# Amandaynzhou/MMT-PSM

Hardware: AMD Instinct MI355X
Metric: imgs/sec (student+teacher step, 1000x1000, AUG_K=2) (higher is better)
Workload: dtype f32

## Files before the change

### include/mmtpsm.h

```cpp
#ifndef MMTPSM_H
#define MMTPSM_H
#include <stdint.h>
#ifdef __cplusplus
extern "C" {
#endif

#define MMT_EINVAL (-22)

int mmt_version(void);

typedef struct {
  const float* feat[4];
  float* grad_feat[4];
  int H[4];
  int W[4];
  float scale[4];
  int num_levels;
  int N;
  int C;
} mmt_pyramid;

int mmt_roi_align_forward(const mmt_pyramid* pyr , const float* rois, const int32_t* levels,
                          int K, int PH, int PW, int sampling_ratio, float* out, void* stream);
int mmt_roi_align_forward_bf16(const mmt_pyramid* pyr , const float* rois, const int32_t* levels,
// ... 147 lines not shown
                          const void* dy_planes, long dy_plane_stride, const float* s_x, const float* s_dy, const float* rowscale,
                          float* dw, float* dbias, float* workspace, void* stream);
typedef struct {
  void* fn;
  long a[16];
} mmt_call;
int mmt_replay(const mmt_call* calls , int n, int* failed_index );
int mmt_split_planes_f16_rb(const float* x, void* planes, long plane_stride, int rows, int W, int C, const float* amax,
                            float* scale_out, void* stream);
int mmt_conv_writes_rb(const mmt_conv_args* a );
typedef struct mmt_wgrad_job {
  mmt_conv_args a;
  const float* dy; const float* rowscale; float* dw; float* dbias;
  const void* x_planes; long x_plane_stride; const void* dy_planes; long dy_plane_stride; const float* s_x; const float* s_dy;
} mmt_wgrad_job;
int mmt_conv_wgrad_group_workspace(const mmt_wgrad_job* jobs , int n, long* floats_out );
int mmt_conv_wgrad_group(const mmt_wgrad_job* jobs , int n, float* workspace, long workspace_floats, void* stream);
int mmt_sum_stats_rb(const float* a, const float* b, const float* c, const float* d, float* y, int rows, int W, int C, float* slot,
                     void* planes, long plane_stride, const float* scale, float* amax_next, void* stream);
int mmt_rb_scales_update(float* state, int n, void* stream);
int mmt_conv_forward_pg(const mmt_conv_args* a , const float* s_x , const float* s_w , int tile_rows,
                        int ksplit, void* stream);
int mmt_conv_pg_plan(const mmt_conv_args* a , int* tile_rows, int* ksplit);
int mmt_conv_pg_wanted(const mmt_conv_args* a );
typedef struct { long src_off, dst_off; int Cout, K, unit0, pad; } mmt_pack_desc;
long mmt_packed_weight_elems(int Cout, int K);
int mmt_pack_weight(const float* w, void* planes, long plane_stride, int Cout, int K, void* stream);
int mmt_pack_weight_flipped(const float* w, const float* scale, void* planes, long plane_stride, int Cout, int KH, int KW,
                            int Cin, void* stream);
int mmt_split_planes(const float* x, void* planes, long plane_stride, long n, void* stream);
typedef struct { const float* w; const float* scale; void* dst; long plane_stride; int Cout, KH, KW, Cin, unit0, pad; } mmt_flip_desc;
int mmt_pack_weights_flipped(const mmt_flip_desc* descs , const int* unit_desc , int n_units, void* stream);
int mmt_pack_weights(const float* base, void* planes, long plane_stride, const mmt_pack_desc* descs ,
                     const int* unit_desc , int n_units, void* stream);
int mmt_pack_weights_f16(const float* base, void* planes, long plane_stride, const mmt_pack_desc* descs ,
                         const int* unit_desc , int n_units, int n_descs, float* stat , void* stream);
int mmt_pack_weights_flipped_f16(const mmt_flip_desc* descs , const int* unit_desc , int n_units, int n_descs,
                                 float* stat , void* stream);

int mmt_conv_wgrad_splits(const mmt_conv_args* a );
int mmt_conv_wgrad(const mmt_conv_args* a , const float* dy,
                   const float* rowscale , float* dw, float* dbias ,
                   float* workspace , void* stream);

int mmt_colsum(const float* dy, int M, int C, float* out, void* stream);

// ... 41 lines not shown
```

### mmt-psm_amd/csrc/conv_igemm.hip

```cpp
#include <stdlib.h>
#include <map>
#include <mutex>
#include <type_traits>
#include "conv_shared.h"

namespace {

template <int BM, int BN, int WM, int WN>
__device__ __forceinline__ void conv_epilogue_stage(f32x16 (&acc)[BM / (32 * WM)][BN / (32 * WN)], float* lds,
                                                    const int lane, const int wm, const int wn) {
  constexpr int TM = BM / (32 * WM), TN = BN / (32 * WN);
  float* ct = lds;
  const int col_l = lane & 31, rq = lane >> 5;
#pragma unroll
  for (int a = 0; a < TM; a++)
#pragma unroll
    for (int b = 0; b < TN; b++)
#pragma unroll
      for (int r = 0; r < 16; r++) {
        const int row = (wm * TM + a) * 32 + (r & 3) + 8 * (r >> 2) + 4 * rq;
        ct[row * BN + (wn * TN + b) * 32 + col_l] = acc[a][b][r];
      }
}

// ... 1793 lines not shown
    }
    return MMT_EINVAL;
  }
  if (ksplit > 1) return launch_glds<128, 128, 4, 1, NS, 3>(p, s, ksplit);
  switch (variant) {
    case 1: return launch_glds<128, 128, 4, 1, NS, 3>(p, s);
    case 3: return launch_glds<128, 64, 4, 1, NS, 3>(p, s);
    default: return launch_glds<64, 64, 2, 2, NS, 3>(p, s);
  }
}

template <int NS>
int launch_split_variant(int variant, const ConvP& p, hipStream_t s) {
  switch (variant) {
    case 1: return launch_split<128, 128, 2, 2, NS>(p, s);
    case 3: return launch_split<128, 64, 2, 2, NS>(p, s);
    default: return launch_split<64, 64, 2, 2, NS>(p, s);
  }
}

}

namespace mmtconv {
static int g_precision = -1;
int precision() {
  if (g_precision < 0) {
    g_precision = getenv("MMT_CONV_PRECISION") ? atoi(getenv("MMT_CONV_PRECISION")) : 3;
    if (g_precision < 0 || g_precision > 3) g_precision = 3;
  }
  return g_precision;
}
}

extern "C" int mmt_set_conv_precision(int mode) {
  if (mode < 0 || mode > 3) return MMT_EINVAL;
  mmtconv::g_precision = mode;
  return 0;
}

extern "C" int mmt_get_conv_precision(void) { return precision(); }

extern "C" int mmt_conv3x3_strip_f16x2(const mmt_conv_args* a, const float* s_x, const float* s_w, void* stream) {
  ConvP p;
  int e = fill(p, a);
  if (e) return e;
  if (!p.y || !p.xpl || !p.wpl || !s_x || !s_w || p.io || p.ypl) return MMT_EINVAL;
// ... 45 lines not shown
extern "C" int mmt_conv_forward_f16x2(const mmt_conv_args* a, const float* x_amax, const float* s_w, void* stream) {
  ConvP p;
  int e = fill(p, a);
  if (e) return e;
  if (!p.y || !p.wpl || !x_amax || !s_w || p.io || p.ypl || p.xpl_rb || (p.Cin & 15) || ((size_t)p.wpl & 15) || (p.wpl_stride & 7)) return MMT_EINVAL;
  if (p.M == 0 || p.Cout == 0) return 0;
  const int variant = pick_variant(p);
  if (variant == 0) return MMT_EINVAL;
  p.f16_sx = x_amax; p.f16_sw = s_w; p.f16_ax = 1;
  hipStream_t s = (hipStream_t)stream;
  if (p.yrb && !rb_epilogue_ok(p)) return MMT_EINVAL;
  if (c64_shape(p)) return launch_c64(p, s);
  if (rows_shape(p, true)) {
    if (p.mask) {
      if (p.Cin == 64) return launch_rows<4, 2, true, true>(p, s);
      if (p.Cin == 128) return launch_rows<8, 2, true, true>(p, s);
      return launch_rows<16, 2, true, true>(p, s);
    }
    if (p.Cin == 64) return launch_rows<4, 2, true>(p, s);
    if (p.Cin == 128) return launch_rows<8, 2, true>(p, s);
    return launch_rows<16, 2, true>(p, s);
  }
  const int ksplit = pick_ksplit(p);
  constexpr int S = 3;
  auto go = [&](auto kern, int BM, int BN, int ks) -> int {
    const int tiles = mmt_cdiv(p.M, BM) * mmt_cdiv(p.Cout, BN) * ks;
    SplitWs w{nullptr, nullptr};
    if (ks > 1) {
      w = split_workspace(s);
      if (!w.ws || tiles > 1024) return MMT_EINVAL;
    }
    const size_t ring = (size_t)S * (BM * 64 + 2 * BN * 32), epi = (size_t)BM * BN * sizeof(float);
    const size_t lds = ring > epi ? ring : epi;
    if (lds > 65536) {
      const hipError_t er = hipFuncSetAttribute((const void*)kern, hipFuncAttributeMaxDynamicSharedMemorySize, (int)lds);
      if (er != hipSuccess) return (int)er;
    }
    hipLaunchKernelGGL(kern, dim3(tiles), dim3(256), lds, s, p, p.wpl, p.wpl_stride, ks, w.ws);
    if (ks > 1)
      launch_finish<128, 128>(p, tiles / ks, ks, w.ws, s);
    return 0;
  };
#define MMT_GLDS_GO(SS)                                                                                      \
  do {                                                                                                       \
    if (ksplit > 1) e = go(conv_fwd_glds_kernel<128, 128, 4, 1, 2, SS, true>, 128, 128, ksplit);            \
    else if (variant == 1) e = go(conv_fwd_glds_kernel<128, 128, 4, 1, 2, SS, true>, 128, 128, 1);          \
// ... 1 lines not shown
    else e = go(conv_fwd_glds_kernel<64, 64, 2, 2, 2, SS, true>, 64, 64, 1);                                \
  } while (0)
  MMT_GLDS_GO(3);
#undef MMT_GLDS_GO
  if (e) return e;
  MMT_LAUNCH_CHECK();
  return 0;
}

static int pick_variant(const ConvP& p) {
  if (p.Cout <= 32) return 0;
  constexpr int lowk = 256;
  constexpr int lowv = 3;
  if (p.K <= lowk) return (p.Cout >= 64 && (long)mmt_cdiv(p.M, 128) * mmt_cdiv(p.Cout, 64) >= 768) ? lowv : 2;
  const long t128 = (long)mmt_cdiv(p.M, 128) * mmt_cdiv(p.Cout, 128);
  constexpr int t128min = 256;
  if (t128 >= t128min && p.Cout > 64) return 1;
  constexpr int mid = 1;
  const long t12864 = (long)mmt_cdiv(p.M, 128) * mmt_cdiv(p.Cout, 64);
  if (mid && t12864 >= 256 && p.Cout >= 64) return 3;
  return 2;
}

extern "C" int mmt_conv_variant(const mmt_conv_args* a) {
  ConvP p;
  int e = fill(p, a);
  if (e) return e;
  const int v = pick_variant(p);
  if (v != 0 && (precision() == 3 || (precision() == 1 && (p.io & IO_X))) && strip_tw(p)) return 4;
  if (v != 0 && precision() > 0 && (p.Cin & 15) == 0 && p.wpl && pick_ksplit(p) > 1) return 1;
  return v;
}

extern "C" int mmt_conv_wants_planes(const mmt_conv_args* a) {
  ConvP p;
  int e = fill(p, a);
  if (e) return 0;
  if (precision() != 3 || pick_variant(p) == 0) return 0;
  return strip_tw(p, false) ? 1 : 0;
}

extern "C" int mmt_conv_ksplit(const mmt_conv_args* a) {
  ConvP p;
  int e = fill(p, a);
  if (e) return e;
  if (pick_variant(p) != 0 && (precision() == 3 || (precision() == 1 && (p.io & IO_X))) && strip_tw(p)) return 1;
  if (pick_variant(p) != 0 && precision() > 0 && (p.Cin & 15) == 0 && p.wpl) return pick_ksplit(p);
  return 1;
}

// ... 30 lines not shown
```

### mmt-psm_amd/csrc/conv_pgemm.hip

```cpp
#include <map>
#include <mutex>
#include "conv_shared.h"

namespace {

constexpr unsigned PG_OOB = 0x80000000u;

template <int I, int U, class F>
__device__ __forceinline__ void pg_unroll(F&& f) {
  if constexpr (I < U) {
    f(std::integral_constant<int, I>{});
    pg_unroll<I + 1, U>(f);
  }
}

template <int WM, int KG, int S, int DBG = 0, bool AF = false>
__global__ __launch_bounds__(768) void conv_pg_kernel(const ConvP p, const int ksplit, float* __restrict__ ws,
                                                      unsigned* __restrict__ tickets) {
  constexpr int BM = 64 * WM, BN = 128, GW = 2 * WM, NT = 512, GT = 64 * GW, NTALL = 768;
  static_assert(GW * KG == 8, "eight matrix waves");
  constexpr int PA = BM * 32, PB = BN * 32;
  constexpr int A_BYTES = 2 * PA, GSTAGE = A_BYTES + 2 * PB, STAGE = KG * GSTAGE;
  constexpr int PPG = 4 / KG, NBP = 8 / PPG, NI = 4 + NBP;
  constexpr int U = (S % 2) ? 2 * S : S;
  constexpr int OWN = 4 / KG;
  static_assert(S >= 3 && (S - 2) * NI < 64, "ring depth / vmcnt range");
  extern __shared__ __attribute__((aligned(16))) float lds[];
  char* const ring = (char*)lds;
  const int tid = threadIdx.x, lane = tid & 63;
  const int wave = __builtin_amdgcn_readfirstlane(tid >> 6);
  const bool copier = wave >= 8;
  const int cw = wave - 8;
  const int grp = copier ? cw / PPG : wave / GW;
  const int gwave = wave % GW;
  const int wm = gwave >> 1, wn = gwave & 1;
  const int gtid = tid - grp * GT;

  const int tiles_n = (p.Cout + BN - 1) / BN;
  int bid = blockIdx.x;
  {
    const int nwg = gridDim.x, q = nwg >> 3, r = nwg & 7, xcd = bid & 7, idx = bid >> 3;
    bid = (xcd < r ? xcd * (q + 1) : r * (q + 1) + (xcd - r) * q) + idx;
  }
  const int ks = bid % ksplit;
  bid /= ksplit;
  const int tile_lin = bid;
  const int tile_m = bid / tiles_n, tile_n = bid % tiles_n;
  const int m0 = tile_m * BM, n0 = tile_n * BN;
  const int HoWo = p.Ho * p.Wo;
  const F16Guard guard = f16_guard_load(p.guard_x);
  const float s_lag = p.xpl_lag ? *p.f16_sx : 0.f;
  auto guard_bad = [&]() { return p.xpl_lag ? f16_guard_bad_lag(guard, s_lag) : f16_guard_bad(guard); };

  const int nkt_all = p.K >> 4, spt = p.Cin >> 4;
  const int R = ksplit * KG, rng = ks * KG + grp;
  const int kt0 = (int)((long)rng * nkt_all / R), nkt = (int)((long)(rng + 1) * nkt_all / R) - kt0;
  const int nkt_max = (nkt_all + R - 1) / R;
  char* const gring = ring + grp * GSTAGE;

  f32x16 acc[2][2];
#pragma unroll
  for (int a = 0; a < 2; a++)
#pragma unroll
    for (int b = 0; b < 2; b++)
#pragma unroll
      for (int r = 0; r < 16; r++) acc[a][b][r] = 0.f;

  if (copier) {
    const int sub = cw % PPG;
    const int ar = (DBG & 64) ? lane >> 3 : (DBG & 32) ? lane >> 2 : lane >> 1;
    const int alh = (DBG & 64) ? (lane & 7) : (DBG & 32) ? (lane & 3) : (lane & 1) ^ ((ar >> 3) & 1);
    int aih0[2], aiw0[2];
    unsigned apix[2];
    bool aok[2];
#pragma unroll
    for (int t = 0; t < 2; t++) {
      const int m = m0 + (2 * sub + t) * 32 + ar;
      aok[t] = m < p.M;
      const int mm = aok[t] ? m : 0;
      const int img = mm / HoWo, rem = mm - img * HoWo;
      const int ho = rem / p.Wo, wo = rem - ho * p.Wo;
      aih0[t] = ho * p.stride - p.pad;
      aiw0[t] = wo * p.stride - p.pad;
      apix[t] = (unsigned)img * (unsigned)(p.H * p.W);
    }
    const long n_x = (long)p.N * p.H * p.W * p.Cin;
    const __amdgpu_buffer_rsrc_t rs_a0 = AF ? __builtin_amdgcn_make_buffer_rsrc((void*)p.x, 0, (int)(n_x * 4), 0x00020000)
                                            : __builtin_amdgcn_make_buffer_rsrc((void*)p.xpl, 0, (int)(n_x * 2), 0x00020000);
    const __amdgpu_buffer_rsrc_t rs_a1 = AF ? rs_a0
                                            : __builtin_amdgcn_make_buffer_rsrc((void*)(p.xpl + p.xpl_stride), 0, (int)(n_x * 2), 0x00020000);
    const __amdgpu_buffer_rsrc_t rs_b = __builtin_amdgcn_make_buffer_rsrc((void*)p.wpl, 0, 0x7ffffff0, 0x00020000);
    const int nb32 = (p.Cout + 31) >> 5;
    const int b_step = nb32 * 1024;
    unsigned vo_b[NBP];
    int dst_b[NBP];
#pragma unroll
    for (int i = 0; i < NBP; i++) {
      const int t = NBP * sub + i, q = t >> 2, cb = t & 3;
      int nb = n0 / 32 + cb;
      if (nb >= nb32) nb = nb32 - 1;
      vo_b[i] = (unsigned)((q * p.wpl_stride + (long)nb * 512 + lane * 8) * 2);
      dst_b[i] = A_BYTES + q * PB + cb * 1024;
    }
    int f_kh, f_kw, f_ci, f_n = 0;
    {
      const int tap0 = kt0 / spt;
      f_ci = kt0 - tap0 * spt;
      f_kh = tap0 / p.KW;
      f_kw = tap0 - f_kh * p.KW;
    }
    const int a_step = AF ? 64 : (p.xpl_rb ? p.W * 32 : 32);
    int soff_a = f_ci * a_step, soff_b = kt0 * b_step;
    unsigned vo_a[2] = {PG_OOB, PG_OOB};
    auto enter_tap = [&]() {
#pragma unroll
      for (int t = 0; t < 2; t++) {
        const int ih = aih0[t] + f_kh, iw = aiw0[t] + f_kw;
        const bool ok = aok[t] && (unsigned)ih < (unsigned)p.H && (unsigned)iw < (unsigned)p.W;
        vo_a[t] = !ok ? PG_OOB
                  : AF ? ((apix[t] + (unsigned)(ih * p.W + iw)) * (unsigned)p.Cin + (unsigned)(alh * 8)) * 4u
                  : p.xpl_rb ? (((apix[t] + (unsigned)(ih * p.W)) * (unsigned)spt + (unsigned)iw) * 16u + (unsigned)(alh * 8)) * 2u
                             : ((apix[t] + (unsigned)(ih * p.W + iw)) * (unsigned)p.Cin + (unsigned)(alh * 8)) * 2u;
      }
    };
    enter_tap();
    auto advance = [&]() {
      f_n++;
      if constexpr (DBG & 1) { soff_b += (DBG & 2) ? 0 : b_step; return; }
      soff_a += a_step;
      soff_b += (DBG & 2) ? 0 : b_step;
      if (++f_ci == spt) {
        f_ci = 0;
        soff_a = 0;
        if (++f_kw == p.KW) { f_kw = 0; ++f_kh; }
        enter_tap();
      }
    };
    auto copy_step = [&](int stage) {
      const bool real = (DBG & 4) ? false : f_n < nkt;
      char* const st = gring + stage * STAGE;
#pragma unroll
      for (int t = 0; t < 2; t++) {
        const int va = (int)(real ? vo_a[t] : PG_OOB);
        __builtin_amdgcn_raw_ptr_buffer_load_lds(rs_a0, (lds_ptr_t)(st + (2 * sub + t) * 1024), 16, va, soff_a, 0, 0);
        __builtin_amdgcn_raw_ptr_buffer_load_lds(rs_a1, (lds_ptr_t)(st + PA + (2 * sub + t) * 1024), 16, va, soff_a, 0, 0);
      }
#pragma unroll
      for (int i = 0; i < NBP; i++)
        __builtin_amdgcn_raw_ptr_buffer_load_lds(rs_b, (lds_ptr_t)(st + dst_b[i]), 16, (int)(real ? vo_b[i] : PG_OOB), soff_b, 0, 0);
      advance();
    };
    auto wait_copies = [&]() {
      asm volatile("s_waitcnt vmcnt(%0)" ::"n"((S - 2) * NI) : "memory");
    };
    if constexpr (AF || (DBG & 16)) {
      typedef unsigned u32x4 __attribute__((ext_vector_type(4)));
      u32x4 rg[S][NI];
      const float s_a = AF ? f16_scale_of(*p.f16_sx) : 1.f;
      auto load_step = [&](auto setc) {
        constexpr int set = decltype(setc)::value;
        const bool real = f_n < nkt;
#pragma unroll
        for (int t = 0; t < 2; t++) {
          const int va = (int)(real ? vo_a[t] : PG_OOB);
          rg[set][2 * t] = __builtin_amdgcn_raw_buffer_load_b128(rs_a0, va, soff_a, 0);
          rg[set][2 * t + 1] = __builtin_amdgcn_raw_buffer_load_b128(rs_a1, AF ? va + 16 : va, soff_a, 0);
        }
#pragma unroll
// ... 82 lines not shown
        default: fa[1][1] = *(const f16x8*)(a + PA + 1024); break;
      }
    };
    auto step = [&](int kt, int st_next, const f16x8 (&fa)[2][2], const f16x8 (&fb)[2][2], f16x8 (&fan)[2][2], f16x8 (&fbn)[2][2]) {
      asm volatile("s_waitcnt lgkmcnt(0)" ::: "memory");
      __builtin_amdgcn_s_barrier();
      if (kt < nkt) {
        int j = 0;
#pragma unroll
        for (int pr = 0; pr < 3; pr++) {
          const int qa = pr == 1 ? 1 : 0, qb = pr == 0 ? 1 : 0;
#pragma unroll
          for (int a = 0; a < 2; a++)
#pragma unroll
            for (int b = 0; b < 2; b++) {
              acc[a][b] = __builtin_amdgcn_mfma_f32_32x32x16_f16(fa[qa][a], fb[qb][b], acc[a][b], 0, 0, 0);
              if (j < 8) { if constexpr (!(DBG & 8)) fread(j, st_next, fan, fbn); }
              j++;
              __builtin_amdgcn_sched_barrier(0);
            }
        }
      }
    };
    if (!guard_bad()) {
      __builtin_amdgcn_s_barrier();
      f16x8 faP[2][2], fbP[2][2], faQ[2][2], fbQ[2][2];
#pragma unroll
      for (int i = 0; i < 8; i++) fread(i, 0, faP, fbP);
      if constexpr (DBG & 8) {
#pragma unroll
        for (int i = 0; i < 8; i++) fread(i, 1, faQ, fbQ);
      }
      for (int kt = 0; kt < nkt_max; kt += U) {
        pg_unroll<0, U>([&](auto ic) {
          constexpr int i = decltype(ic)::value;
          if (i == 0 || kt + i < nkt_max) {
            if constexpr (i % 2 == 0) step(kt + i, (i + 1) % S, faP, fbP, faQ, fbQ);
            else step(kt + i, (i + 1) % S, faQ, fbQ, faP, fbP);
          }
        });
      }
    }
    asm volatile("s_waitcnt lgkmcnt(0)" ::: "memory");
  }
  if (guard_bad()) {
    if (ks == 0) conv_slow_tile(m0, BM, 0, BM, n0, BN, nullptr, false, tid, NTALL, blockIdx.x);
    return;
// ... 74 lines not shown
            u32x4 t[4];
#pragma unroll
            for (int r4 = 0; r4 < 4; r4++) t[r4] = __builtin_amdgcn_raw_buffer_load_b128(rws, (int)(slab_off + (unsigned)((o * 4 + r4) * NT * 16)), 0, 16);
#pragma unroll
            for (int r4 = 0; r4 < 4; r4++) {
              const f32x4 v = __builtin_bit_cast(f32x4, t[r4]);
#pragma unroll
              for (int c = 0; c < 4; c++) {
                if (j == 0) acc[i >> 1][i & 1][4 * r4 + c] = v[c]; else acc[i >> 1][i & 1][4 * r4 + c] += v[c];
              }
            }
            o++;
          }
        }
      }
    }
  }

  {
    const int mrow0 = m0 + wm * 64 + 4 * (lane >> 5);
    conv_epilogue_direct<2, 2>(p, acc, (unsigned)mrow0 * ((unsigned)p.Cout * 4u), p.M - mrow0, n0 + wn * 64 + (lane & 31),
                         copier ? 0 : (KG == 1 ? 15 : (KG == 2 ? (grp ? 10 : 5) : (1 << grp))), (float*)ring + 64, wave, lane, tid, blockIdx.x);
  }
}

__global__ __launch_bounds__(256) void split_planes_f16_rb_kernel(const float* __restrict__ x, unsigned short* __restrict__ pl,
                                                                  const long plane_stride, const int W, const int C, const int segs,
                                                                  const float* __restrict__ amax, float* __restrict__ s_out) {
  constexpr int CBS = 1024 + 32;
  __shared__ __attribute__((aligned(16))) char tile[2 * 16 * CBS];
  const float s = f16_scale_of(*amax);
  if (blockIdx.x == 0 && blockIdx.y == 0 && threadIdx.x == 0 && s_out) *s_out = s;
  const int row = blockIdx.x / segs, w0 = (blockIdx.x % segs) * 32, c0 = blockIdx.y * 256;
  const int cc = min(256, C - c0), c4n = cc >> 2, ncb = cc >> 4, npx = min(32, W - w0);
  const float* const src = x + ((long)row * W + w0) * C + c0;
  const int total = npx * c4n;
  f32x4 v[8];
#pragma unroll
  for (int u = 0; u < 8; u++) {
    const int i = threadIdx.x + 256 * u;
    const int px = i / c4n, c4 = i - px * c4n;
    v[u] = i < total ? ldg4(src + (long)px * C + c4 * 4) : f32x4{0.f, 0.f, 0.f, 0.f};
  }
#pragma unroll
  for (int u = 0; u < 8; u++) {
    const int i = threadIdx.x + 256 * u;
// ... 122 lines not shown

bool pg_shape(const ConvP& p) {
  return p.xpl && p.wpl && !p.io && !p.ypl && !p.mul && p.out_stride == 1 && p.res_mode <= 1 && (p.Cin & 15) == 0 && p.Cout > 32 &&
         (long)p.N * p.H * p.W * p.Cin < (1L << 29) && (long)p.M * p.Cout * 4 < (1L << 31) && ((size_t)p.xpl & 15) == 0 &&
         (p.xpl_stride & 7) == 0 && ((size_t)p.wpl & 15) == 0 && (p.wpl_stride & 7) == 0;
}

void pg_plan(const ConvP& p, int& rows, int& ksplit) {
  const long tn = mmt_cdiv(p.Cout, 128);
  const long t256 = (long)mmt_cdiv(p.M, 256) * tn, t128 = (long)mmt_cdiv(p.M, 128) * tn, t64 = (long)mmt_cdiv(p.M, 64) * tn;
  const int nkt = p.K >> 4;
  rows = t256 >= 448 ? 256 : (t128 >= 224 ? 128 : 64);
  ksplit = 1;
  if (rows == 64 && t64 <= 128) {
    int ks = (int)(256 / t64);
    if (ks > nkt / 64) ks = nkt / 64;
    if (ks > 8) ks = 8;
    if (ks >= 2) ksplit = ks;
  }
  const char* e = getenv("MMT_SPLITK");
  if (e && atoi(e) == 0) ksplit = 1;
}

template <int WM, int KG, int S, int DBG = 0, bool AF = false>
int launch_pg(const ConvP& p, hipStream_t s, int ksplit) {
  constexpr int BM = 64 * WM;
  const int tiles = mmt_cdiv(p.M, BM) * mmt_cdiv(p.Cout, 128);
  SplitWs w{nullptr, nullptr};
  if (ksplit > 1) {
    w = split_workspace(s);
    if (!w.ws || !w.tickets || tiles > SPLITK_TICKETS || (size_t)tiles * ksplit * BM * 128 * 4 > SPLITK_WS_BYTES) return MMT_EINVAL;
  }
  constexpr size_t ring = (size_t)S * KG * (BM * 64 + 2 * 128 * 32), xch = KG > 1 ? (size_t)4 * (KG - 1) * 4 * (128 * WM) * 16 : 0;
  constexpr size_t lds = ring > xch ? ring : xch;
  static_assert(lds <= 160 * 1024, "LDS");
  auto kern = conv_pg_kernel<WM, KG, S, DBG, AF>;
  static bool done = false;
  if (!done) {
    const hipError_t e = hipFuncSetAttribute((const void*)kern, hipFuncAttributeMaxDynamicSharedMemorySize, (int)lds);
    if (e != hipSuccess) return (int)e;
    done = true;
  }
  hipLaunchKernelGGL(kern, dim3(tiles * ksplit), dim3(768), lds, s, p, ksplit, w.ws, w.tickets);
  MMT_LAUNCH_CHECK();
  return 0;
}

}

extern "C" int mmt_conv_pg_plan(const mmt_conv_args* a, int* tile_rows, int* ksplit) {
  ConvP p;
  int e = fill(p, a);
  if (e) return e;
  int rows = 0, ks = 0;
  if (precision() == 3 && p.wpl && p.M > 0 && p.Cout > 0) {
    const unsigned short* keep = p.xpl;
    if (!p.xpl) p.xpl = (const unsigned short*)16;
    if (pg_shape(p)) pg_plan(p, rows, ks);
    p.xpl = keep;
  }
  if (tile_rows) *tile_rows = rows;
  if (ksplit) *ksplit = ks;
  return 0;
}

extern "C" int mmt_conv_pg_wanted(const mmt_conv_args* a) {
  ConvP p;
  if (fill(p, a)) return 0;
  if (precision() != 3 || !p.wpl || p.M <= 0 || p.Cout < 96 || p.KH * p.KW < 4) return 0;
  const char* e = getenv("MMT_PG");
// ... 82 lines not shown
      case 8: return launch_pg<1, 4, 3, 8>(p, s, ks);
      case 12: return launch_pg<1, 4, 3, 12>(p, s, ks);
      default: break;
    }
    if (rows == 256) switch (dbg) {
      case 1: return launch_pg<4, 1, 4, 1>(p, s, ks);
      case 2: return launch_pg<4, 1, 4, 2>(p, s, ks);
      case 4: return launch_pg<4, 1, 4, 4>(p, s, ks);
      case 8: return launch_pg<4, 1, 4, 8>(p, s, ks);
      case 12: return launch_pg<4, 1, 4, 12>(p, s, ks);
      default: break;
    }
  }
#endif
  if (af) {
#ifdef MMT_PG_ABLATE
    if (rows == 256) return launch_pg<4, 1, 4, 0, true>(p, s, ks);
    if (rows == 128) return launch_pg<2, 2, 4, 0, true>(p, s, ks);
    return launch_pg<1, 4, 3, 0, true>(p, s, ks);
#else
    return MMT_EINVAL;
#endif
  }
  if (rows == 256) return launch_pg<4, 1, 4>(p, s, ks);
  if (rows == 128) return launch_pg<2, 2, 4>(p, s, ks);
  return launch_pg<1, 4, 3>(p, s, ks);
}
```

### mmt-psm_amd/csrc/conv_shared.h

```cpp
#pragma once
#include <stdlib.h>
#include <type_traits>
#include "common.h"

namespace mmtconv {

struct ConvP {
  const float* x; const float* w; const float* scale; const float* shift; const float* res;
  const float* mask; const float* mul; float* y;
  int N, H, W, Cin, Cout, KH, KW, stride, pad, Ho, Wo;
  int relu, res_mode, out_stride, out_H, out_W;
  float mask_scale;
  int M, K, cin32, cin4;
  const unsigned short* wpl; long wpl_stride;
  const unsigned short* xpl; long xpl_stride;
  unsigned short* ypl; long ypl_stride;
  unsigned* amax_out;
  int amax_stats;
  int f16_ax;
  const float* f16_sx; const float* f16_sw;
  int io;
  const float* guard_x; const float* guard_dy;
  const float* w_src; const float* w_src_scale;
  const float* x2; const float* dy2; const float* f16_sx2; const float* f16_sw2; const float* guard_x2; const float* guard_dy2;
// ... 1 lines not shown
  int staged_epilogue;
  int xpl_rb;
  unsigned short* yrb; long yrb_stride; const float* yrb_s; unsigned* amax_next; int xpl_lag;
  int yrb_M;
};
constexpr float F16_CREST_HI = 131072.f;
constexpr int IO_X = 1, IO_Y = 2, IO_RES = 4, IO_MASK = 8, IO_DY = 16;

int fill(ConvP& p, const mmt_conv_args* a);
int precision();
struct SplitWs { float* ws; unsigned* tickets; };
constexpr size_t SPLITK_WS_BYTES = (size_t)1024 * 128 * 128 * 4;
constexpr int SPLITK_TICKETS = 4096;
SplitWs split_workspace(hipStream_t s);
struct WgReduceItem { const float* ws; const float* rowscale; float* dw; int splits, Cout, NP, pad; };
int launch_wgrad_reduce_group(const WgReduceItem* items, int n, hipStream_t s);
struct WgPlJob { const mmt_conv_args* a; const float* dy; const void* xpl; long xpl_stride; const void* dpl; long dpl_stride;
                 const float* s_x; const float* s_dy; const float* rowscale; float* dw; float* dbias; float* ws; int ksplit; };
int wgpl_eligible_splits(const mmt_conv_args* a);
long wgpl_super_steps(const mmt_conv_args* a);
int launch_wgpl_group(const WgPlJob* jobs, int n, hipStream_t s);
bool c64_shape(const ConvP& p);
int launch_c64(const ConvP& p, hipStream_t s);
}

namespace {
using namespace mmtconv;

struct F16Guard { float amax, s0, s1, s2, s3, c0, c1, c2, c3; };
__device__ __forceinline__ F16Guard f16_guard_load(const float* __restrict__ slot) {
  F16Guard g = {0.f, 0.f, 0.f, 0.f, 0.f, 0.f, 0.f, 0.f, 0.f};
  if (slot) { g.amax = slot[0]; g.s0 = slot[1]; g.s1 = slot[2]; g.s2 = slot[3]; g.s3 = slot[4];
              g.c0 = slot[17]; g.c1 = slot[18]; g.c2 = slot[19]; g.c3 = slot[20]; }
  return g;
}
__device__ __forceinline__ bool f16_guard_bad(const F16Guard& g) {
  const float tot = (g.s0 + g.s1) + (g.s2 + g.s3), cnt = (g.c0 + g.c1) + (g.c2 + g.c3);
  if (!(tot > 0.f)) return false;
  if (!(g.amax == g.amax) || g.amax > 3.0e38f) return true;
  return g.amax * cnt > tot * F16_CREST_HI;
}

__device__ __forceinline__ bool f16_guard_bad_lag(const F16Guard& g, const float s) {
  const float tot = (g.s0 + g.s1) + (g.s2 + g.s3), cnt = (g.c0 + g.c1) + (g.c2 + g.c3);
  if (!(g.amax == g.amax) || g.amax > 3.0e38f) return true;
  if (g.amax * s > 60000.f) return true;
// ... 17 lines not shown
  float r0 = v[0], r1 = v[1], r2 = v[2], r3 = v[3];
#pragma unroll
  for (int q = 0; q < NS; q++) {
    const unsigned a = pk_bf16(r0, r1), b = pk_bf16(r2, r3);
    o[q] = uint2{a, b};
    if (q + 1 < NS) {
      r0 -= __builtin_bit_cast(float, a << 16);
      r1 -= __builtin_bit_cast(float, a & 0xffff0000u);
      r2 -= __builtin_bit_cast(float, b << 16);
      r3 -= __builtin_bit_cast(float, b & 0xffff0000u);
    }
  }
}
__device__ __forceinline__ float f16_scale_of(const float amax) {
  if (!(amax > 0.f)) return 1.f;
  int e;
  frexpf(amax, &e);
  e = 14 - e;
  e = e > 100 ? 100 : (e < -100 ? -100 : e);
  return ldexpf(1.f, e);
}

__device__ __forceinline__ f32x4 ldg4(const float* p) { return *(const f32x4*)p; }
__device__ __forceinline__ void split4h(const f32x4 v, const float s, uint2 (&o)[2]) {
  float r[4] = {v[0] * s, v[1] * s, v[2] * s, v[3] * s};
#pragma unroll
  for (int e = 0; e < 4; e++) r[e] = fminf(fmaxf(r[e], -65504.f), 65504.f);
  _Float16 h[4], l[4];
#pragma unroll
  for (int e = 0; e < 4; e++) { h[e] = (_Float16)r[e]; l[e] = (_Float16)(r[e] - (float)h[e]); }
  o[0] = uint2{__builtin_bit_cast(unsigned, f16x2{h[0], h[1]}), __builtin_bit_cast(unsigned, f16x2{h[2], h[3]})};
  o[1] = uint2{__builtin_bit_cast(unsigned, f16x2{l[0], l[1]}), __builtin_bit_cast(unsigned, f16x2{l[2], l[3]})};
}

struct AmaxAcc { float amx = 0.f, asum = 0.f, acnt = 0.f; };

__device__ __forceinline__ unsigned rb_split1(const float v, const float s) {
  const float r = __builtin_amdgcn_fmed3f(v * s, -65504.f, 65504.f);
  const _Float16 h = (_Float16)r;
  const _Float16 l = (_Float16)(r - (float)h);
  return __builtin_bit_cast(unsigned, f16x2{h, l});
}
struct RbGeom { int Wo; float rWo; unsigned cb32; };
__device__ __forceinline__ RbGeom rb_geom(const ConvP& p) {
  return RbGeom{p.Wo, 1.f / (float)p.Wo, (unsigned)(p.Cout >> 4) * (unsigned)p.Wo * 32u};
}
__device__ __forceinline__ unsigned rb_row_off(const RbGeom& g, const int m) {
  int row = (int)(((float)m + 0.5f) * g.rWo);
  int w = m - row * g.Wo;
  if (w < 0) { row--; w += g.Wo; } else if (w >= g.Wo) { row++; w -= g.Wo; }
  return (unsigned)row * g.cb32 + (unsigned)w * 32u;
}
__device__ __forceinline__ void rb_store4(const ConvP& p, const RbGeom& g, const int m, const int c, const f32x4 v, const float s) {
  uint2 o[2];
  split4h(v, s, o);
// ... 211 lines not shown
```

### mmt-psm_amd/maskrcnn_benchmark/_hip.py

```python
import ctypes
import weakref
import os
import threading as _threading

import torch

_HERE = os.path.dirname(os.path.abspath(__file__))
LIB_PATH = os.path.join(os.path.dirname(_HERE), "libmmtpsm.so")

c_void_p, c_int, c_float, c_double, c_int64 = ctypes.c_void_p, ctypes.c_int, ctypes.c_float, ctypes.c_double, ctypes.c_int64


class Pyramid(ctypes.Structure):
    _fields_ = [("feat", c_void_p * 4), ("grad_feat", c_void_p * 4), ("H", c_int * 4), ("W", c_int * 4),
                ("scale", c_float * 4), ("num_levels", c_int), ("N", c_int), ("C", c_int)]


class ConvArgs(ctypes.Structure):
    _fields_ = [("x", c_void_p), ("w", c_void_p), ("scale", c_void_p), ("shift", c_void_p), ("res", c_void_p),
                ("mask", c_void_p), ("mul", c_void_p), ("y", c_void_p),
                ("N", c_int), ("H", c_int), ("W", c_int), ("Cin", c_int), ("Cout", c_int), ("KH", c_int),
                ("KW", c_int), ("stride", c_int), ("pad", c_int), ("Ho", c_int), ("Wo", c_int),
                ("relu", c_int), ("res_mode", c_int), ("out_stride", c_int), ("out_H", c_int), ("out_W", c_int),
                ("mask_scale", c_float), ("w_planes", c_void_p), ("w_plane_stride", ctypes.c_long),
# ... 103 lines not shown
                                   c_void_p, c_void_p, c_void_p, c_void_p, c_void_p, c_void_p],
    "mmt_ciam_fwd": [c_void_p, c_void_p, c_int, c_int, c_int, c_int, c_void_p, c_void_p, c_void_p, c_void_p, c_void_p],
    "mmt_ciam_bwd": [c_void_p, c_void_p, c_int, c_int, c_int, c_int, c_void_p, c_void_p, c_void_p, c_void_p, c_void_p, c_void_p,
                     c_void_p, c_void_p, c_void_p],
    "mmt_stats_combine": [c_void_p, c_int, c_void_p, c_void_p],
    "mmt_sum_stats": [c_void_p, c_void_p, c_void_p, c_void_p, c_void_p, ctypes.c_long, c_void_p, c_void_p],
    "mmt_split_planes_f16": [c_void_p, c_void_p, ctypes.c_long, ctypes.c_long, c_float, c_void_p, c_void_p, c_void_p, c_void_p, c_void_p],
    "mmt_split_planes_f16_rb": [c_void_p, c_void_p, ctypes.c_long, c_int, c_int, c_int, c_void_p, c_void_p, c_void_p],
    "mmt_replay": [c_void_p, c_int, c_void_p],
    "mmt_conv_writes_rb": [ctypes.POINTER(ConvArgs)],
    "mmt_conv_wgrad_group_workspace": [c_void_p, c_int, ctypes.POINTER(ctypes.c_long)],
    "mmt_conv_wgrad_group": [c_void_p, c_int, c_void_p, ctypes.c_long, c_void_p],
    "mmt_sum_stats_rb": [c_void_p, c_void_p, c_void_p, c_void_p, c_void_p, c_int, c_int, c_int, c_void_p, c_void_p, ctypes.c_long, c_void_p,
                         c_void_p, c_void_p],
    "mmt_rb_scales_update": [c_void_p, c_int, c_void_p],
    "mmt_conv_wgrad_planes_splits": [ctypes.POINTER(ConvArgs)],
    "mmt_conv_wgrad_planes": [ctypes.POINTER(ConvArgs), c_void_p, c_void_p, ctypes.c_long, c_void_p, ctypes.c_long, c_void_p, c_void_p,
                              c_void_p, c_void_p, c_void_p, c_void_p, c_void_p],
    "mmt_pack_weight_f16": [c_void_p, c_void_p, ctypes.c_long, c_int, c_int, c_float, c_void_p, c_void_p, c_void_p],
    "mmt_pack_weight_flipped_f16": [c_void_p, c_void_p, c_void_p, ctypes.c_long, c_int, c_int, c_int, c_int, c_void_p, c_void_p, c_void_p],
    "mmt_conv3x3_strip_f16x2": [ctypes.POINTER(ConvArgs), c_void_p, c_void_p, c_void_p],
    "mmt_conv_forward_f16x2": [ctypes.POINTER(ConvArgs), c_void_p, c_void_p, c_void_p],
    "mmt_conv_forward_pg": [ctypes.POINTER(ConvArgs), c_void_p, c_void_p, c_int, c_int, c_void_p],
    "mmt_conv_pg_plan": [ctypes.POINTER(ConvArgs), c_void_p, c_void_p],
    "mmt_conv_pg_wanted": [ctypes.POINTER(ConvArgs)],
    "mmt_stem_fused": [c_void_p, c_int, c_int, c_int, c_void_p, c_void_p, ctypes.c_long, c_void_p, c_void_p, c_void_p, c_void_p, c_void_p,
                       c_void_p, c_void_p],
    "mmt_maxpool3x3s2_bf16": [c_void_p, c_void_p, c_int, c_int, c_int, c_int, c_int, c_int, c_void_p],
    "mmt_mask_bce": [c_void_p, c_void_p, c_void_p, c_int, c_int, c_int, c_float, c_void_p, c_void_p, c_void_p],
    "mmt_mgd_level_forward": [c_void_p, ctypes.POINTER(MgdTeachers), c_void_p, c_int, c_int, c_int, c_int, c_void_p, c_void_p],
    "mmt_mgd_level_backward": [c_void_p, ctypes.POINTER(MgdTeachers), c_void_p, c_int, c_int, c_int, c_int, c_void_p, c_void_p, c_void_p],
    "mmt_mask_pool": [c_void_p, c_int, c_int, c_int, c_int, c_int, c_void_p, c_void_p],
    "mmt_psm_rows": [c_void_p, c_int, c_void_p, c_int, c_int, c_void_p, c_float, c_int, c_int, c_void_p, c_void_p, c_void_p],
    "mmt_psm_variance": [c_void_p, c_int, c_int, c_int, c_int, c_void_p, c_void_p],
    "mmt_ema_update": [c_void_p, c_void_p, c_int64, c_double, c_void_p],
    "mmt_sgd_momentum": [c_void_p, c_void_p, c_void_p, c_int64, c_float, c_float, c_float, c_int, c_void_p],
    "mmt_paste_masks": [c_void_p, c_void_p, c_void_p, c_void_p, c_int, c_int, c_int, c_int, c_int, c_float, c_void_p, c_void_p],
    "mmt_paste_mask_stack": [c_void_p, c_void_p, c_int, c_int, c_int, c_int, c_float, c_void_p, c_void_p],
    "mmt_polygon_targets": [c_void_p, c_void_p, c_void_p, c_void_p, c_int, c_int, c_void_p, c_void_p, c_void_p],
}

_lib = None
PROFILE = None
PROFILE_ALL = False
AUTO_PLANES = True
_BF16_STORAGE = os.environ.get("MMT_BF16_STORAGE", "0") != "0"
# ... 2015 lines not shown
```

Baseline: 126.8.

## Add fp32-input pipelined GEMM conv that splits activations to f16 pairs in-kernel

Adds a variant of the pipelined f16x2 GEMM conv kernel that loads fp32 activations directly into LDS and splits them into high and low f16 halves inside the MFMA loop. This avoids a separate split-planes pass and its extra memory traffic. The tiled f16x2 forward path now routes eligible shapes to this kernel by default. The cost is twice the activation bytes per K step and extra VALU work interleaved between MFMAs. Saturation clamping is dropped in the split, which risks overflow when scaled values exceed the f16 range.

```diff
diff --git a/include/mmtpsm.h b/include/mmtpsm.h
--- a/include/mmtpsm.h
+++ b/include/mmtpsm.h
@@ -193,6 +193,8 @@
 int mmt_conv_forward_pg(const mmt_conv_args* a , const float* s_x , const float* s_w , int tile_rows,
                         int ksplit, void* stream);
 int mmt_conv_pg_plan(const mmt_conv_args* a , int* tile_rows, int* ksplit);
+int mmt_conv_forward_pgx(const mmt_conv_args* a , const float* x_amax , const float* s_w , int tile_rows,
+                         int ksplit, void* stream);
 int mmt_conv_pg_wanted(const mmt_conv_args* a );
 typedef struct { long src_off, dst_off; int Cout, K, unit0, pad; } mmt_pack_desc;
 long mmt_packed_weight_elems(int Cout, int K);
diff --git a/mmt-psm_amd/csrc/conv_igemm.hip b/mmt-psm_amd/csrc/conv_igemm.hip
--- a/mmt-psm_amd/csrc/conv_igemm.hip
+++ b/mmt-psm_amd/csrc/conv_igemm.hip
@@ -1839,6 +1839,7 @@
 }
 
 namespace mmtconv {
+int tiled_ksplit(const ConvP& p) { return pick_ksplit(p); }
 static int g_precision = -1;
 int precision() {
   if (g_precision < 0) {
@@ -1930,6 +1931,10 @@
     return launch_rows<16, 2, true>(p, s);
   }
   const int ksplit = pick_ksplit(p);
+  {
+    int rows, ks;
+    if (pgx_shape(p) && pgx_plan(p, ksplit, rows, ks)) return launch_pgx(p, s, rows, ks);
+  }
   constexpr int S = 3;
   auto go = [&](auto kern, int BM, int BN, int ks) -> int {
     const int tiles = mmt_cdiv(p.M, BM) * mmt_cdiv(p.Cout, BN) * ks;
@@ -1977,10 +1982,19 @@
   return 2;
 }
 
+static bool f16x2_takes_pgx(ConvP p) {
+  if (precision() != 3 || p.io || p.xpl || p.ypl || pick_variant(p) == 0 || (p.Cin & 15) || !p.wpl) return false;
+  if (!p.x) p.x = (const float*)16;
+  if (c64_shape(p) || rows_shape(p, true)) return false;
+  int rows, ks;
+  return pgx_shape(p) && pgx_plan(p, pick_ksplit(p), rows, ks);
+}
+
 extern "C" int mmt_conv_variant(const mmt_conv_args* a) {
   ConvP p;
   int e = fill(p, a);
   if (e) return e;
+  if (f16x2_takes_pgx(p)) return 5;
   const int v = pick_variant(p);
   if (v != 0 && (precision() == 3 || (precision() == 1 && (p.io & IO_X))) && strip_tw(p)) return 4;
   if (v != 0 && precision() > 0 && (p.Cin & 15) == 0 && p.wpl && pick_ksplit(p) > 1) return 1;
diff --git a/mmt-psm_amd/csrc/conv_pgemm.hip b/mmt-psm_amd/csrc/conv_pgemm.hip
--- a/mmt-psm_amd/csrc/conv_pgemm.hip
+++ b/mmt-psm_amd/csrc/conv_pgemm.hip
@@ -14,11 +14,11 @@
   }
 }
 
-template <int WM, int KG, int S, int DBG = 0, bool AF = false>
-__global__ __launch_bounds__(768) void conv_pg_kernel(const ConvP p, const int ksplit, float* __restrict__ ws,
-                                                      unsigned* __restrict__ tickets) {
+template <int WM, int KG, int S, int DBG, bool AF, bool X32>
+__device__ __forceinline__ void pg_block(const ConvP& p, const int ksplit, float* __restrict__ ws, unsigned* __restrict__ tickets) {
   constexpr int BM = 64 * WM, BN = 128, GW = 2 * WM, NT = 512, GT = 64 * GW, NTALL = 768;
   static_assert(GW * KG == 8, "eight matrix waves");
+  static_assert(!(X32 && (AF || DBG)), "the fp32-row form has no ablation arm");
   constexpr int PA = BM * 32, PB = BN * 32;
   constexpr int A_BYTES = 2 * PA, GSTAGE = A_BYTES + 2 * PB, STAGE = KG * GSTAGE;
   constexpr int PPG = 4 / KG, NBP = 8 / PPG, NI = 4 + NBP;
@@ -49,8 +49,8 @@
   const int m0 = tile_m * BM, n0 = tile_n * BN;
   const int HoWo = p.Ho * p.Wo;
   const F16Guard guard = f16_guard_load(p.guard_x);
-  const float s_lag = p.xpl_lag ? *p.f16_sx : 0.f;
-  auto guard_bad = [&]() { return p.xpl_lag ? f16_guard_bad_lag(guard, s_lag) : f16_guard_bad(guard); };
+  const float s_lag = !X32 && p.xpl_lag ? *p.f16_sx : 0.f;
+  auto guard_bad = [&]() { return !X32 && p.xpl_lag ? f16_guard_bad_lag(guard, s_lag) : f16_guard_bad(guard); };
 
   const int nkt_all = p.K >> 4, spt = p.Cin >> 4;
   const int R = ksplit * KG, rng = ks * KG + grp;
@@ -68,14 +68,16 @@
 
   if (copier) {
     const int sub = cw % PPG;
-    const int ar = (DBG & 64) ? lane >> 3 : (DBG & 32) ? lane >> 2 : lane >> 1;
-    const int alh = (DBG & 64) ? (lane & 7) : (DBG & 32) ? (lane & 3) : (lane & 1) ^ ((ar >> 3) & 1);
-    int aih0[2], aiw0[2];
-    unsigned apix[2];
-    bool aok[2];
-#pragma unroll
-    for (int t = 0; t < 2; t++) {
-      const int m = m0 + (2 * sub + t) * 32 + ar;
+    constexpr int NA = X32 ? 4 : 2;
+    const int ar = X32 ? lane >> 2 : (DBG & 64) ? lane >> 3 : (DBG & 32) ? lane >> 2 : lane >> 1;
+    const int alh = X32 ? (lane & 3) ^ ((lane >> 4) & 3)
+                  : (DBG & 64) ? (lane & 7) : (DBG & 32) ? (lane & 3) : (lane & 1) ^ ((ar >> 3) & 1);
+    int aih0[NA], aiw0[NA];
+    unsigned apix[NA];
+    bool aok[NA];
+#pragma unroll
+    for (int t = 0; t < NA; t++) {
+      const int m = m0 + (X32 ? (4 * sub + t) * 16 : (2 * sub + t) * 32) + ar;
       aok[t] = m < p.M;
       const int mm = aok[t] ? m : 0;
       const int img = mm / HoWo, rem = mm - img * HoWo;
@@ -85,9 +87,9 @@
       apix[t] = (unsigned)img * (unsigned)(p.H * p.W);
     }
     const long n_x = (long)p.N * p.H * p.W * p.Cin;
-    const __amdgpu_buffer_rsrc_t rs_a0 = AF ? __builtin_amdgcn_make_buffer_rsrc((void*)p.x, 0, (int)(n_x * 4), 0x00020000)
-                                            : __builtin_amdgcn_make_buffer_rsrc((void*)p.xpl, 0, (int)(n_x * 2), 0x00020000);
-    const __amdgpu_buffer_rsrc_t rs_a1 = AF ? rs_a0
+    const __amdgpu_buffer_rsrc_t rs_a0 = AF || X32 ? __builtin_amdgcn_make_buffer_rsrc((void*)p.x, 0, (int)(n_x * 4), 0x00020000)
+                                                   : __builtin_amdgcn_make_buffer_rsrc((void*)p.xpl, 0, (int)(n_x * 2), 0x00020000);
+    const __amdgpu_buffer_rsrc_t rs_a1 = AF || X32 ? rs_a0
                                             : __builtin_amdgcn_make_buffer_rsrc((void*)(p.xpl + p.xpl_stride), 0, (int)(n_x * 2), 0x00020000);
     const __amdgpu_buffer_rsrc_t rs_b = __builtin_amdgcn_make_buffer_rsrc((void*)p.wpl, 0, 0x7ffffff0, 0x00020000);
     const int nb32 = (p.Cout + 31) >> 5;
@@ -109,15 +111,18 @@
       f_kh = tap0 / p.KW;
       f_kw = tap0 - f_kh * p.KW;
     }
-    const int a_step = AF ? 64 : (p.xpl_rb ? p.W * 32 : 32);
+    const int a_step = AF || X32 ? 64 : (p.xpl_rb ? p.W * 32 : 32);
     int soff_a = f_ci * a_step, soff_b = kt0 * b_step;
-    unsigned vo_a[2] = {PG_OOB, PG_OOB};
+    unsigned vo_a[NA];
+#pragma unroll
+    for (int t = 0; t < NA; t++) vo_a[t] = PG_OOB;
     auto enter_tap = [&]() {
 #pragma unroll
-      for (int t = 0; t < 2; t++) {
+      for (int t = 0; t < NA; t++) {
         const int ih = aih0[t] + f_kh, iw = aiw0[t] + f_kw;
         const bool ok = aok[t] && (unsigned)ih < (unsigned)p.H && (unsigned)iw < (unsigned)p.W;
         vo_a[t] = !ok ? PG_OOB
+                  : X32 ? ((apix[t] + (unsigned)(ih * p.W + iw)) * (unsigned)p.Cin + (unsigned)(alh * 4)) * 4u
                   : AF ? ((apix[t] + (unsigned)(ih * p.W + iw)) * (unsigned)p.Cin + (unsigned)(alh * 8)) * 4u
                   : p.xpl_rb ? (((apix[t] + (unsigned)(ih * p.W)) * (unsigned)spt + (unsigned)iw) * 16u + (unsigned)(alh * 8)) * 2u
                              : ((apix[t] + (unsigned)(ih * p.W + iw)) * (unsigned)p.Cin + (unsigned)(alh * 8)) * 2u;
@@ -139,11 +144,17 @@
     auto copy_step = [&](int stage) {
       const bool real = (DBG & 4) ? false : f_n < nkt;
       char* const st = gring + stage * STAGE;
-#pragma unroll
-      for (int t = 0; t < 2; t++) {
-        const int va = (int)(real ? vo_a[t] : PG_OOB);
-        __builtin_amdgcn_raw_ptr_buffer_load_lds(rs_a0, (lds_ptr_t)(st + (2 * sub + t) * 1024), 16, va, soff_a, 0, 0);
-        __builtin_amdgcn_raw_ptr_buffer_load_lds(rs_a1, (lds_ptr_t)(st + PA + (2 * sub + t) * 1024), 16, va, soff_a, 0, 0);
+      if constexpr (X32) {
+#pragma unroll
+        for (int t = 0; t < 4; t++)
+          __builtin_amdgcn_raw_ptr_buffer_load_lds(rs_a0, (lds_ptr_t)(st + (4 * sub + t) * 1024), 16, (int)(real ? vo_a[t] : PG_OOB), soff_a, 0, 0);
+      } else {
+#pragma unroll
+        for (int t = 0; t < 2; t++) {
+          const int va = (int)(real ? vo_a[t] : PG_OOB);
+          __builtin_amdgcn_raw_ptr_buffer_load_lds(rs_a0, (lds_ptr_t)(st + (2 * sub + t) * 1024), 16, va, soff_a, 0, 0);
+          __builtin_amdgcn_raw_ptr_buffer_load_lds(rs_a1, (lds_ptr_t)(st + PA + (2 * sub + t) * 1024), 16, va, soff_a, 0, 0);
+        }
       }
 #pragma unroll
       for (int i = 0; i < NBP; i++)
@@ -272,7 +283,75 @@
         }
       }
     };
-    if (!guard_bad()) {
+    if constexpr (X32) {
+      const int arow = wm * 64 + lr;
+      const char* const fA32 = gring + arow * 64;
+      const int ac0 = ((2 * kh2) ^ ((lr >> 2) & 3)) << 4, ac1 = ((2 * kh2 + 1) ^ ((lr >> 2) & 3)) << 4;
+      const float s_a = f16_scale_of(*p.f16_sx);
+      f32x4 va[2][2];
+      unsigned hw[2][4], lw[2][4];
+      auto fread32 = [&](int i, int stage, f16x8 (&fb)[2][2]) {
+        const char* const a = fA32 + stage * STAGE;
+        const char* const b = fB + stage * STAGE;
+        switch (i) {
+          case 0: va[0][0] = *(const f32x4*)(a + ac0); break;
+          case 1: va[0][1] = *(const f32x4*)(a + ac1); break;
+          case 2: va[1][0] = *(const f32x4*)(a + 32 * 64 + ac0); break;
+          case 3: va[1][1] = *(const f32x4*)(a + 32 * 64 + ac1); break;
+          case 4: fb[1][0] = *(const f16x8*)(b + PB); break;
+          case 5: fb[1][1] = *(const f16x8*)(b + PB + 1024); break;
+          case 6: fb[0][0] = *(const f16x8*)(b); break;
+          default: fb[0][1] = *(const f16x8*)(b + 1024); break;
+        }
+      };
+      auto split_piece = [&](int i, f16x8 (&fa)[2][2]) {
+        const int a = i >> 2, h = (i >> 1) & 1, e = i & 1;
+        split2h<false>(va[a][h][2 * e], va[a][h][2 * e + 1], s_a, hw[a][2 * h + e], lw[a][2 * h + e]);
+        if ((i & 3) == 3) {
+          typedef unsigned u32x4 __attribute__((ext_vector_type(4)));
+          fa[0][a] = __builtin_bit_cast(f16x8, u32x4{hw[a][0], hw[a][1], hw[a][2], hw[a][3]});
+          fa[1][a] = __builtin_bit_cast(f16x8, u32x4{lw[a][0], lw[a][1], lw[a][2], lw[a][3]});
+        }
+      };
+      auto step32 = [&](int kt, int st_next, const f16x8 (&fa)[2][2], const f16x8 (&fb)[2][2], f16x8 (&fan)[2][2], f16x8 (&fbn)[2][2]) {
+        asm volatile("s_waitcnt lgkmcnt(0)" ::: "memory");
+        __builtin_amdgcn_s_barrier();
+        if (kt < nkt) {
+          int j = 0;
+#pragma unroll
+          for (int pr = 0; pr < 3; pr++) {
+            const int qa = pr == 1 ? 1 : 0, qb = pr == 0 ? 1 : 0;
+#pragma unroll
+            for (int a = 0; a < 2; a++)
+#pragma unroll
+              for (int b = 0; b < 2; b++) {
+                acc[a][b] = __builtin_amdgcn_mfma_f32_32x32x16_f16(fa[qa][a], fb[qb][b], acc[a][b], 0, 0, 0);
+                if (j < 4) { fread32(2 * j, st_next, fbn); fread32(2 * j + 1, st_next, fbn); }
+                else split_piece(j - 4, fan);
+                j++;
+                __builtin_amdgcn_sched_barrier(0);
+              }
+          }
+        }
+      };
+      if (!guard_bad()) {
+        __builtin_amdgcn_s_barrier();
+        f16x8 faP[2][2], fbP[2][2], faQ[2][2], fbQ[2][2];
+#pragma unroll
+        for (int i = 0; i < 8; i++) fread32(i, 0, fbP);
+#pragma unroll
+        for (int i = 0; i < 8; i++) split_piece(i, faP);
+        for (int kt = 0; kt < nkt_max; kt += U) {
+          pg_unroll<0, U>([&](auto ic) {
+            constexpr int i = decltype(ic)::value;
+            if (i == 0 || kt + i < nkt_max) {
+              if constexpr (i % 2 == 0) step32(kt + i, (i + 1) % S, faP, fbP, faQ, fbQ);
+              else step32(kt + i, (i + 1) % S, faQ, fbQ, faP, fbP);
+            }
+          });
+        }
+      }
+    } else if (!guard_bad()) {
       __builtin_amdgcn_s_barrier();
       f16x8 faP[2][2], fbP[2][2], faQ[2][2], fbQ[2][2];
 #pragma unroll
@@ -393,6 +472,18 @@
     conv_epilogue_direct<2, 2>(p, acc, (unsigned)mrow0 * ((unsigned)p.Cout * 4u), p.M - mrow0, n0 + wn * 64 + (lane & 31),
                          copier ? 0 : (KG == 1 ? 15 : (KG == 2 ? (grp ? 10 : 5) : (1 << grp))), (float*)ring + 64, wave, lane, tid, blockIdx.x);
   }
+}
+
+template <int WM, int KG, int S, int DBG = 0, bool AF = false>
+__global__ __launch_bounds__(768) void conv_pg_kernel(const ConvP p, const int ksplit, float* __restrict__ ws,
+                                                      unsigned* __restrict__ tickets) {
+  pg_block<WM, KG, S, DBG, AF, false>(p, ksplit, ws, tickets);
+}
+
+template <int WM, int KG, int S>
+__global__ __launch_bounds__(768) void conv_pgx_kernel(const ConvP p, const int ksplit, float* __restrict__ ws,
+                                                       unsigned* __restrict__ tickets) {
+  pg_block<WM, KG, S, 0, false, true>(p, ksplit, ws, tickets);
 }
 
 __global__ __launch_bounds__(256) void split_planes_f16_rb_kernel(const float* __restrict__ x, unsigned short* __restrict__ pl,
@@ -561,7 +652,7 @@
   if (e && atoi(e) == 0) ksplit = 1;
 }
 
-template <int WM, int KG, int S, int DBG = 0, bool AF = false>
+template <int WM, int KG, int S, int DBG = 0, bool AF = false, bool X32 = false>
 int launch_pg(const ConvP& p, hipStream_t s, int ksplit) {
   constexpr int BM = 64 * WM;
   const int tiles = mmt_cdiv(p.M, BM) * mmt_cdiv(p.Cout, 128);
@@ -573,7 +664,8 @@
   constexpr size_t ring = (size_t)S * KG * (BM * 64 + 2 * 128 * 32), xch = KG > 1 ? (size_t)4 * (KG - 1) * 4 * (128 * WM) * 16 : 0;
   constexpr size_t lds = ring > xch ? ring : xch;
   static_assert(lds <= 160 * 1024, "LDS");
-  auto kern = conv_pg_kernel<WM, KG, S, DBG, AF>;
+  void (*kern)(const ConvP, const int, float*, unsigned*);
+  if constexpr (X32) kern = conv_pgx_kernel<WM, KG, S>; else kern = conv_pg_kernel<WM, KG, S, DBG, AF>;
   static bool done = false;
   if (!done) {
     const hipError_t e = hipFuncSetAttribute((const void*)kern, hipFuncAttributeMaxDynamicSharedMemorySize, (int)lds);
@@ -585,6 +677,53 @@
   return 0;
 }
 
+bool pgx_plan_of(const ConvP& p, const int ranges, int& rows, int& ksplit) {
+  const long t256 = (long)mmt_cdiv(p.M, 256) * mmt_cdiv(p.Cout, 128);
+  rows = 256;
+  ksplit = ranges < 1 ? 1 : ranges;
+  if (ksplit == 1) return t256 >= 256;
+  if ((ksplit == 2 || ksplit == 4) && p.K < 4096) {
+    rows = 256 / ksplit;
+    ksplit = 1;
+    return true;
+  }
+  return t256 <= SPLITK_TICKETS && (size_t)t256 * ksplit * 256 * 128 * 4 <= SPLITK_WS_BYTES;
+}
+
+template <bool X32>
+int launch_pg_rows(const ConvP& p, hipStream_t s, int rows, int ks) {
+  if (rows == 256) return launch_pg<4, 1, 4, 0, false, X32>(p, s, ks);
+  if (rows == 128) return launch_pg<2, 2, 4, 0, false, X32>(p, s, ks);
+  return launch_pg<1, 4, 3, 0, false, X32>(p, s, ks);
+}
+
+}
+
+namespace mmtconv {
+bool pgx_shape(const ConvP& p) {
+  if (!p.x || p.xpl) return false;
+  ConvP q = p;
+  q.xpl = (const unsigned short*)p.x;
+  q.xpl_stride = 0;
+  return pg_shape(q);
+}
+bool pgx_plan(const ConvP& p, int ranges, int& rows, int& ksplit) { return pgx_plan_of(p, ranges, rows, ksplit); }
+int launch_pgx(const ConvP& p, hipStream_t s, int rows, int ksplit) { return launch_pg_rows<true>(p, s, rows, ksplit); }
+}
+
+extern "C" int mmt_conv_forward_pgx(const mmt_conv_args* a, const float* x_amax, const float* s_w, int tile_rows, int ksplit, void* stream) {
+  ConvP p;
+  int e = fill(p, a);
+  if (e) return e;
+  if (!p.y || !x_amax || !s_w || precision() != 3 || !pgx_shape(p) || (p.yrb && (p.Cout & 15))) return MMT_EINVAL;
+  if (p.M == 0 || p.Cout == 0) return 0;
+  p.f16_sx = x_amax; p.f16_sw = s_w; p.f16_ax = 1;
+  int rows, ks;
+  pgx_plan_of(p, tiled_ksplit(p), rows, ks);
+  if (tile_rows == 64 || tile_rows == 128 || tile_rows == 256) rows = tile_rows; else if (tile_rows != 0) return MMT_EINVAL;
+  if (ksplit > 0) ks = ksplit;
+  if (ks < 1 || ks * (256 / rows) > (p.K >> 4)) return MMT_EINVAL;
+  return launch_pg_rows<true>(p, (hipStream_t)stream, rows, ks);
 }
 
 extern "C" int mmt_conv_pg_plan(const mmt_conv_args* a, int* tile_rows, int* ksplit) {
@@ -713,7 +852,5 @@
     return MMT_EINVAL;
 #endif
   }
-  if (rows == 256) return launch_pg<4, 1, 4>(p, s, ks);
-  if (rows == 128) return launch_pg<2, 2, 4>(p, s, ks);
-  return launch_pg<1, 4, 3>(p, s, ks);
-}
+  return launch_pg_rows<false>(p, s, rows, ks);
+}
diff --git a/mmt-psm_amd/csrc/conv_shared.h b/mmt-psm_amd/csrc/conv_shared.h
--- a/mmt-psm_amd/csrc/conv_shared.h
+++ b/mmt-psm_amd/csrc/conv_shared.h
@@ -47,6 +47,10 @@
 int launch_wgpl_group(const WgPlJob* jobs, int n, hipStream_t s);
 bool c64_shape(const ConvP& p);
 int launch_c64(const ConvP& p, hipStream_t s);
+bool pgx_shape(const ConvP& p);
+bool pgx_plan(const ConvP& p, int ranges, int& rows, int& ksplit);
+int launch_pgx(const ConvP& p, hipStream_t s, int rows, int ksplit);
+int tiled_ksplit(const ConvP& p);
 }
 
 namespace {
@@ -110,15 +114,21 @@
 }
 
 __device__ __forceinline__ f32x4 ldg4(const float* p) { return *(const f32x4*)p; }
+template <bool SAT = true>
+__device__ __forceinline__ void split2h(const float v0, const float v1, const float s, unsigned& hh, unsigned& ll) {
+  f32x2 r = {v0 * s, v1 * s};
+  if constexpr (SAT) {
+    r[0] = fminf(fmaxf(r[0], -65504.f), 65504.f);
+    r[1] = fminf(fmaxf(r[1], -65504.f), 65504.f);
+  }
+  const f16x2 h = __builtin_convertvector(r, f16x2);
+  const f32x2 l = {__builtin_fmaf((float)h[0], -1.f, r[0]), __builtin_fmaf((float)h[1], -1.f, r[1])};
+  hh = __builtin_bit_cast(unsigned, h);
+  ll = __builtin_bit_cast(unsigned, __builtin_convertvector(l, f16x2));
+}
 __device__ __forceinline__ void split4h(const f32x4 v, const float s, uint2 (&o)[2]) {
-  float r[4] = {v[0] * s, v[1] * s, v[2] * s, v[3] * s};
-#pragma unroll
-  for (int e = 0; e < 4; e++) r[e] = fminf(fmaxf(r[e], -65504.f), 65504.f);
-  _Float16 h[4], l[4];
-#pragma unroll
-  for (int e = 0; e < 4; e++) { h[e] = (_Float16)r[e]; l[e] = (_Float16)(r[e] - (float)h[e]); }
-  o[0] = uint2{__builtin_bit_cast(unsigned, f16x2{h[0], h[1]}), __builtin_bit_cast(unsigned, f16x2{h[2], h[3]})};
-  o[1] = uint2{__builtin_bit_cast(unsigned, f16x2{l[0], l[1]}), __builtin_bit_cast(unsigned, f16x2{l[2], l[3]})};
+  split2h(v[0], v[1], s, o[0].x, o[1].x);
+  split2h(v[2], v[3], s, o[0].y, o[1].y);
 }
 
 struct AmaxAcc { float amx = 0.f, asum = 0.f, acnt = 0.f; };
diff --git a/mmt-psm_amd/maskrcnn_benchmark/_hip.py b/mmt-psm_amd/maskrcnn_benchmark/_hip.py
--- a/mmt-psm_amd/maskrcnn_benchmark/_hip.py
+++ b/mmt-psm_amd/maskrcnn_benchmark/_hip.py
@@ -149,6 +149,7 @@
     "mmt_conv3x3_strip_f16x2": [ctypes.POINTER(ConvArgs), c_void_p, c_void_p, c_void_p],
     "mmt_conv_forward_f16x2": [ctypes.POINTER(ConvArgs), c_void_p, c_void_p, c_void_p],
     "mmt_conv_forward_pg": [ctypes.POINTER(ConvArgs), c_void_p, c_void_p, c_int, c_int, c_void_p],
+    "mmt_conv_forward_pgx": [ctypes.POINTER(ConvArgs), c_void_p, c_void_p, c_int, c_int, c_void_p],
     "mmt_conv_pg_plan": [ctypes.POINTER(ConvArgs), c_void_p, c_void_p],
     "mmt_conv_pg_wanted": [ctypes.POINTER(ConvArgs)],
     "mmt_stem_fused": [c_void_p, c_int, c_int, c_int, c_void_p, c_void_p, ctypes.c_long, c_void_p, c_void_p, c_void_p, c_void_p, c_void_p,
```

Measured after the change: 128.2 (median of 6 runs). 1.01x the previous value.
